# KarelPeeters/kZero

Hardware: AMD Instinct MI355X
Metric: self-play NN evals/sec (node), Chess 20x256 ResNet b=256, 1/2/4/8 GPU (higher is better)
Workload: dtype f16; 1 GPU; chess-20x256 attention head, executor batch 256; engines_per_gpu=1, parallelism=dp1 (no collective)

## Files before the change

### kzero_amd/csrc/kz_decode_dev.hpp

```cpp
#pragma once

struct DecodeDev {
    const int64_t *move_offsets;
    const int32_t *move_indices;
    float *values;
    float *probs;
    int *error_flag;
    int policy_len;
    const uint8_t *sym = nullptr;
    const int32_t *policy_map = nullptr;
    int n_sym = 0;
};

inline DecodeDev decode_dev(const DecodeArgs &a, bool on, int policy_len) {
    return DecodeDev{on ? a.move_offsets : nullptr, a.move_indices, a.values, a.probs, a.error_flag, policy_len, a.sym, a.policy_map, a.n_sym};
}

__device__ __forceinline__ float decode_wave_max_nan(float v) {
#pragma unroll
    for (int off = 32; off > 0; off >>= 1) {
        const float o = __shfl_xor(v, off, 64);
        v = (v != v || o != o) ? NAN : fmaxf(v, o);
    }
    return v;
}

__device__ __forceinline__ void decode_raise(const DecodeDev &d, int board) {
    *reinterpret_cast<volatile int *>(d.error_flag) = 1;
    raise_decode_board(d.error_flag, board);
}

__device__ __forceinline__ float decode_wave_sum(float v) {
#pragma unroll
    for (int off = 32; off > 0; off >>= 1) v += __shfl_xor(v, off, 64);
    return v;
}

template <class LogitAt>
__device__ __forceinline__ void decode_board_wave(const DecodeDev &d, int board, int lane, const float *raw, float *stage,
                                                  int cap, LogitAt logit_at) {
    if (lane == 0) {
        const float s0 = raw[0], s1 = raw[1], s2 = raw[2], s3 = raw[3], s4 = raw[4];
        const float m = fmaxf(s1, fmaxf(s2, s3));
        const float e0 = expf(s1 - m), e1 = expf(s2 - m), e2 = expf(s3 - m), sum = e0 + e1 + e2;
        float *v = d.values + (size_t)board * 5;
        v[0] = tanhf(s0);
        v[1] = e0 / sum;
        v[2] = e1 / sum;
        v[3] = e2 / sum;
        v[4] = s4;
        if (!(sum > 0.0f)) decode_raise(d, board);
    }
    const int64_t lo = d.move_offsets[board];
    const int n = (int)(d.move_offsets[board + 1] - lo);
    const int32_t *pmap = nullptr;
    if (d.sym) {
        const int id = d.sym[board];
        if (id < d.n_sym) pmap = d.policy_map + (size_t)id * d.policy_len;
        else if (lane == 0) decode_raise(d, board);
    }
    if (n <= 0) return;
    auto logit_of = [&](int i) {
        int idx = d.move_indices[lo + i];
        if (d.sym) idx = (pmap && idx >= 0 && idx < d.policy_len) ? pmap[idx] : -1;
        return (idx >= 0 && idx < d.policy_len) ? logit_at(idx) : NAN;
    };
    float mx = -INFINITY;
    for (int i = lane; i < n; i += 64) {
        const float v = logit_of(i);
        if (i < cap) stage[i] = v;
        mx = (mx != mx || v != v) ? NAN : fmaxf(mx, v);
    }
    mx = decode_wave_max_nan(mx);
    float sum = 0.0f;
    for (int i = lane; i < n; i += 64) {
        const float e = expf((i < cap ? stage[i] : logit_of(i)) - mx);
        if (i < cap) stage[i] = e;
        sum += e;
    }
    sum = decode_wave_sum(sum);
    if (lane == 0 && !(sum > 0.0f)) decode_raise(d, board);
    for (int i = lane; i < n; i += 64) d.probs[lo + i] = (i < cap ? stage[i] : expf(logit_of(i) - mx)) / sum;
}
```

### kzero_amd/csrc/kz_encode_dev.hpp

```cpp
#pragma once

__device__ __forceinline__ float encoded_plane(const PackedBoards in, int board, int ch, int square, int hw) {
    float f = 0.0f;
    if (ch < in.n_scalar) {
        f = in.scalars[(size_t)board * in.n_scalar + ch];
    } else if (ch < in.n_scalar + in.n_bool) {
        const uint8_t *bb = in.bits + (size_t)board * in.stride;
        if (in.sym) square = in.square_src[min((int)in.sym[board], in.n_sym - 1) * hw + square];
        const unsigned bit = (unsigned)(ch - in.n_scalar) * hw + square;
        f = (float)((bb[bit >> 3] >> (bit & 7)) & 1);
    }
    return f;
}
```

### kzero_amd/csrc/kz_engine.hip

```cpp
#include <hip/hip_runtime.h>

#include <algorithm>
#include <cmath>
#include <cstdio>
#include <cstdlib>
#include <cstring>
#include <map>
#include <memory>
#include <mutex>
#include <stdexcept>
#include <string>
#include <tuple>
#include <vector>

#include "../../include/kz_hip.h"
#include "kz_kernels.hpp"
#include "kz_model.hpp"

namespace {

#include "kz_engine_util.hpp"
#include "kz_plan.hpp"
#include "kz_device_weights.hpp"

#include "kz_engine_state.hpp"
#include "kz_engine_forward.hpp"

static void experiment_switches(const Model &m, int dtype, int cin_p, PathPlan &p) {
#ifdef KZ_EXPERIMENTS
    const auto env_int = [](const char *name) { return getenv(name) ? atoi(getenv(name)) : 0; };
    if (env_on("KZ_NO_TOWER_F16") && p.tower == Tower::resident_f16) {
        p.tower = kz::tower_split_supported(m.h, m.w, m.channels, m.depth, m.c_in, false) ? Tower::resident_f16g : Tower::conv_igemm;
        p.heads = p.wide = false;
    }
    p.nb4 = p.tower == Tower::resident_f16 && env_int("KZ_TOWER_NB") == 4 && cin_p == 32;
    if (p.nb4) p.heads = false;
    p.tower_prev = p.tower == Tower::resident_f16 && !p.nb4 && env_on("KZ_TOWER_PREV");
    p.t32_dense3 = p.tower == Tower::resident_f32 && env_int("KZ_T32_BOARDS") == 3 &&
                   kz::tower32_dense3_supported((int)m.policy_kind, m.policy_extra_moves, m.policy_conv_channels, m.h, m.w, m.channels,
                                                m.sh_conv.cout, m.sh_fc0.out, p.heads);
    p.att_heads = !p.heads && att_heads_one_launch(m, dtype);
    p.conv2 = env_on("KZ_BOARD_CONV2") && p.tower == Tower::board_conv_f16 &&
              kz::board_conv2_supported(dtype, m.h, m.w, m.channels, m.channels);
    p.graph = env_on("KZ_HIP_GRAPH") && !p.heads;
    p.no_zero_copy = env_on("KZ_NO_ZERO_COPY");
#endif
}

static void launch_geometry_of(const Model &m, const PathPlan &p, int dtype, int batch, int *workgroups, int *boards_per_workgroup) {
    const int cin_p = round_up(m.c_in, 32), cp = round_up(m.channels, 32);
    int per = 0, wgs = 0;
    switch (p.tower) {
// ... 1468 lines not shown
    return guarded("kz_memcpy_d2h", [&]() -> int {
        HIP_TRY(hipSetDevice(device));
        HIP_TRY(hipMemcpy(dst, src, bytes, hipMemcpyDeviceToHost));
        return 0;
    });
}

KZ_API int kz_device_synchronize(int device) {
    return guarded("kz_device_synchronize", [&]() -> int {
        HIP_TRY(hipSetDevice(device));
        HIP_TRY(hipDeviceSynchronize());
        return 0;
    });
}

KZ_API int kz_engine_set_profiling(kz_engine *e, int enable) {
    return guarded("kz_engine_set_profiling", [&]() -> int {
        if (!e) return fail("kz_engine_set_profiling: null engine");
        HIP_TRY(hipSetDevice(e->device));
        if (e->sync_all()) return 1;
        e->prof.clear();
        e->prof.on = enable != 0;
        return 0;
    });
}

KZ_API int kz_engine_kernel_time(kz_engine *e, const char *prefix, double *total_ms, int64_t *launches) {
    return guarded("kz_engine_kernel_time", [&]() -> int {
        if (!e || !prefix || !total_ms || !launches) return fail("kz_engine_kernel_time: null argument");
        HIP_TRY(hipSetDevice(e->device));
// ... 55 lines not shown
```

### kzero_amd/csrc/kz_engine_forward.hpp

```cpp
#pragma once

inline int kz_engine::conv(const Pass &p, const DevConv &w, const void *x, int ldx, void *y, int ldy, int M, int relu, const void *res, bool post,
         int h, int wd, int group, int src_group, int src_off, float *y32, int ldy32) {
    if (w.bws) {
        kz::BoardConvArgs b{};
        b.x = x; b.ldx = 2 * ldx; b.weights = w.bws; b.bias = w.b; b.res = res; b.y = y; b.ldy = 2 * ldy;
        b.y32 = y32; b.ldy32 = ldy32;
        b.post_scale = post ? wts->post_scale : nullptr;
        b.post_shift = post ? wts->post_shift : nullptr;
        b.boards = M / (h * wd); b.h = h; b.w = wd; b.cin = w.cin_p; b.cout = w.cout; b.relu = relu;
        return launch(p, "kz_board_conv_split16", [&] { kz::launch_board_conv_split(b, p.stream); });
    }
    if (w.bw) {
        kz::BoardConvArgs b{};
        b.x = x; b.ldx = ldx; b.weights = w.bw; b.bias = w.b; b.res = res; b.y = y; b.ldy = ldy;
        b.post_scale = post ? wts->post_scale : nullptr;
        b.post_shift = post ? wts->post_shift : nullptr;
        b.boards = M / (h * wd); b.h = h; b.w = wd; b.cin = w.cin_p; b.cout = w.cout; b.relu = relu;
        b.rowmap = wts->bc_rowmap; b.halo = wts->bc_halo; b.n_halo = wts->bc_n_halo;
        return launch(p, "kz_board_conv_f16", [&] {
#ifdef KZ_EXPERIMENTS
            if (w.bw2) kz::launch_board_conv2(b, p.stream);
            else
#endif
// ... 61 lines not shown
        t.x0 = x_in; t.cin_p = cin_p; t.w_stem = wts->res.w_stem; t.w_tower = wts->res.w_tower;
        t.bias = wts->res.bias; t.post_scale = wts->post_scale; t.post_shift = wts->post_shift;
        t.y = act[0]; t.batch = batch; t.h = m.h; t.w = m.w; t.depth = m.depth;
        t.boards_per_wg = plan.tower_nb;
        t.fused_heads = plan.heads;
        t.sh_w0 = wts->sh.w0; t.sh_b0 = wts->sh.b0; t.sh_w1 = wts->sh.w1; t.sh_b1 = wts->sh.b1;
        t.sh_w2 = wts->sh.w2; t.sh_b2 = wts->sh.b2; t.att_idx = wts->res.att_idx;
        t.scalars = d_scalars; t.policy = d_policy;
        t.nonfinite_flag = p.nf_flag; t.epoch = p.nf_epoch;
        if (dec && plan.heads) t.decode = *dec;
        if (tap_out) {
            t.taps = taps();
            range_site = 2 * m.depth + 1;
        }
#ifdef KZ_EXPERIMENTS
        t.prev = plan.tower_prev;
#endif
        if (launch(p, "kz_tower_resident_f16", [&] {
#ifdef KZ_EXPERIMENTS
                if (plan.nb4) kz::launch_tower_resident4(t, xres, p.stream);
                else
#endif
                kz::launch_tower_resident(t, p.stream);
            }))
            return 1;
        tower_out = 0;
        return 0;
    }
    if (!per_layer(plan)) {
        kz::Tower32Args t{};
        t.x0 = (const float *)x_in; t.ldx0 = cin_p; t.c_in = m.c_in; t.weights = wts->res.w32; t.bias = wts->res.bias;
// ... 231 lines not shown
```

### kzero_amd/csrc/kz_kernels.hpp

```cpp
#pragma once
#include <vector>
#include <hip/hip_runtime.h>

#include <cstdint>

namespace kz {

inline int round_up(int v, int m) { return (v + m - 1) / m * m; }

constexpr int ERR_HDR = 4;
inline size_t error_flag_words(int max_batch) { return ERR_HDR + 2 * (size_t)max_batch; }
__device__ __forceinline__ void raise_nonfinite_board(int *nonfinite_flag, int epoch, int board) {
    *reinterpret_cast<volatile int *>(nonfinite_flag - 1 - board) = epoch;
}
__device__ __forceinline__ void raise_decode_board(int *error_flag, int board) {
    *reinterpret_cast<volatile int *>(error_flag + ERR_HDR + 2 * board) = 1;
}

struct PackedBoards {
    const uint8_t *bits = nullptr;
    size_t stride = 0;
    const float *scalars = nullptr;
    int n_scalar = 0, n_bool = 0;
    int n_sym = 0;
// ... 364 lines not shown
    const void *w_stem;
    const void *w_tower;
    const float *bias;
    const float *post_scale, *post_shift;
    void *y;
    int batch, h, w, depth;
    int boards_per_wg;
    bool fused_heads;
    const float *sh_w0, *sh_b0, *sh_w1, *sh_b1, *sh_w2, *sh_b2;
    const int32_t *att_idx;
    float *scalars, *policy;
    int *nonfinite_flag;
    int epoch;
    DecodeArgs decode;
    bool prev;
    TapOut taps;
};
bool tower_resident_supported(int dtype, int h, int w, int channels, int depth, int c_in);
bool tower_heads_supported(int policy_kind, int query_channels, int policy_len, int sh_channels, int sh_size);
size_t tower_packed_weight_elems(int cin_p, int depth);
size_t tower_heads_weight_elems();
size_t tower_weight_pad_elems();
void tower_pack_heads(const float *w_bulk, const float *b_bulk, const float *w_under, const float *b_under,
                      uint16_t *dst, float *bias5);
void tower_pack_weights(const float *oihw, int cout, int cin, int cin_p, uint16_t *dst, bool tap_major = false);
void launch_tower_resident(const TowerArgs &a, hipStream_t stream);
size_t tower4_scratch_bytes(int batch);
void launch_tower_resident4(const TowerArgs &a, void *xres, hipStream_t stream);

}
```

### kzero_amd/csrc/kz_plan.hpp

```cpp
#pragma once


enum class Tower {
    dense_net,
    att_valu,
    att_mfma,
    resident_f16,
    resident_f32,
    resident_split16,
    resident_f16g,
    resident_bf16g,
    resident_i8,
    board_conv_f16,
    board_conv_split16,
    conv_igemm,
};

struct PathPlan {
    Tower tower = Tower::conv_igemm;
    bool heads = false;
    bool wide = false;
    int wide_cap = 0;
    bool att_heads = false;
    bool keep = false;
    int tower_nb = 2;
    int launches = 0;
#ifdef KZ_EXPERIMENTS
    bool nb4 = false, tower_prev = false, t32_dense3 = false, conv2 = false, graph = false, no_zero_copy = false;
#endif
};

bool split_arithmetic(Tower t) { return t == Tower::resident_split16 || t == Tower::board_conv_split16; }
bool split_arithmetic(const PathPlan &p) { return split_arithmetic(p.tower); }

enum class StreamHeads { none, attention, conv };
struct WeightsSpec {
    Tower tower = Tower::conv_igemm;
    StreamHeads heads = StreamHeads::none;
    bool att_heads = false;
    bool conv2 = false, nb4 = false;
    auto fields() const { return std::tie(tower, heads, att_heads, conv2, nb4); }
    bool operator<(const WeightsSpec &o) const { return fields() < o.fields(); }
};
// ... 241 lines not shown
```

### kzero_amd/csrc/kz_tower.hip

```cpp
#include <cstdlib>
#include <type_traits>
#include <vector>

#include "kz_kernels.hpp"
#include "kz_launch.hpp"
#include "kz_tower_boundary.hpp"
namespace kz {

typedef _Float16 h16;
typedef h16 h16x8 __attribute__((ext_vector_type(8)));
typedef h16 h16x4 __attribute__((ext_vector_type(4)));
typedef float f32x4 __attribute__((ext_vector_type(4)));

namespace {

#include "kz_decode_dev.hpp"
#include "kz_encode_dev.hpp"

constexpr int C = 256;
constexpr int RS = C * 2 + 16;
constexpr int URS = 3 * C * 2 + 16;
constexpr int KSTEPS = 72;
constexpr int HEAD_KSTEPS = 5 * 8;
constexpr int POLICY = 1880, LOGIT_LD = 96;
constexpr int TOWER_PF_MAX = 8;

struct TowerDev {
    const h16 *x0;
    const uint4 *w_stem, *w_tower;
    const float *bias, *post_scale, *post_shift;
    h16 *y;
    int cin_p, batch, depth;
    PackedBoards in;
    const float *sh_w0, *sh_b0, *sh_w1, *sh_b1, *sh_w2, *sh_b2;
    const int32_t *att_idx;
    union { float *scalars; unsigned char *tap_base; }; union { float *policy; size_t tap_site_bytes; };
    int *nonfinite_flag;
    int epoch;
    DecodeDev dec;
};

template <int I, int N, class F>
__device__ __forceinline__ void static_for(F &&f) {
    if constexpr (I < N) {
        f(std::integral_constant<int, I>{});
        static_for<I + 1, N>(f);
    }
}

template <int NB>
struct Layout {
    static constexpr int M = NB * 64;
    static constexpr int MT = M / 16;
    static constexpr bool LINE_TILES = NB == 2;
    static constexpr int BPAD = LINE_TILES ? 128 : 0;
    static constexpr int BOARD = 64 * RS + BPAD;
    static constexpr int TS = LINE_TILES ? 8 * RS : 16 * RS;
    static constexpr int IMG = NB * BOARD;
    static constexpr int X_OFF = 0;
    static constexpr int Y_OFF = IMG;
    static constexpr int Z_OFF = 2 * IMG;
    static_assert(Z_OFF % 256 == 0, "zero rows keep the slot pattern of the image rows");
    static constexpr int S_OFF = Z_OFF + 16 * RS;
    static constexpr int TOWER_BYTES = S_OFF + M * 64;
    static constexpr int U_OFF = Z_OFF;
    static constexpr int ACT_OFF = U_OFF + 16 * URS;
    static constexpr int HID_OFF = ACT_OFF + NB * 256 * 4;
    static constexpr int HEADS_BYTES = HID_OFF + NB * 32 * 4;
    static constexpr int LOG_OFF = Y_OFF;
    static constexpr int BYTES = TOWER_BYTES > HEADS_BYTES ? TOWER_BYTES : HEADS_BYTES;
    static_assert(NB * 64 * LOGIT_LD * 4 <= IMG, "logits fit the Y region");
    static constexpr int row_off(int b, int p) { return b * BOARD + p * RS; }
    static_assert(BYTES <= 160 * 1024, "LDS budget");
};

constexpr int SG_VALU = 0x2, SG_SALU = 0x4, SG_MFMA = 0x8, SG_VMEM_READ = 0x20, SG_DS_READ = 0x100;

template <int NB, bool HEADS, int PF, bool WIDE = false, bool PREV = false, bool TAP = false>
__global__ __launch_bounds__(256, 1) void kz_tower_resident(TowerDev a) {
    using L = Layout<NB>;
    constexpr int M = L::M, MT = L::MT;
    static_assert(PF <= TOWER_PF_MAX, "the refills past the end of the stream must land in its padding"); static_assert(!TAP || (!HEADS && !PREV), "the tap instances are the plain tower's");
    extern __shared__ __attribute__((aligned(16))) unsigned char lds[];

    const int tid = threadIdx.x;
    const int wave = __builtin_amdgcn_readfirstlane(tid >> 6);
    const int lane = tid & 63;
    const int fr = lane & 15, kq = lane >> 4;
    const int board0 = blockIdx.x * NB;
    const int layers = 2 * a.depth;
    const int total_ksteps = layers * KSTEPS + (HEADS ? HEAD_KSTEPS : 0);
    const int bias_rows = layers + (HEADS ? 5 : 0);

    const uint4 *wp = a.w_tower + wave * 256 + lane;
    auto wload_prev = [&](int gk, int nt) __attribute__((always_inline)) { return wp[(size_t)gk * 1024 + nt * 64]; };
    typedef const __attribute__((address_space(1))) unsigned char *gptr;
    gptr wk = (gptr)a.w_tower + wave * 4096;
    const unsigned wlane = lane * 16;
    auto wload = [&](gptr k, int nt) __attribute__((always_inline)) {
        typedef unsigned u32x4 __attribute__((ext_vector_type(4)));
        return __builtin_bit_cast(uint4, *reinterpret_cast<const __attribute__((address_space(1))) u32x4 *>(k + wlane + nt * 1024));
    };
    uint4 wreg[PF][4];
#pragma unroll
    for (int s = 0; s < PF; s++) {
        const int g = s < total_ksteps ? s : total_ksteps - 1;
#pragma unroll
        for (int nt = 0; nt < 4; nt++) wreg[s][nt] = PREV ? wload_prev(g, nt) : wload(wk + s * 16384, nt);
    }
    wk += PF * 16384;
    int g = 0;
    auto ring_take = [&](int stage, h16x8 (&af)[4]) __attribute__((always_inline)) {
#pragma unroll
        for (int nt = 0; nt < 4; nt++) af[nt] = *reinterpret_cast<const h16x8 *>(&wreg[stage][nt]);
#ifndef KZ_TW_NO_WLOAD
        if constexpr (PREV) {
            const int gn = g + PF < total_ksteps ? g + PF : total_ksteps - 1;
#pragma unroll
            for (int nt = 0; nt < 4; nt++) wreg[stage][nt] = wload_prev(gn, nt);
        } else {
#pragma unroll
            for (int nt = 0; nt < 4; nt++) wreg[stage][nt] = wload(wk, nt);
        }
#endif
        wk += 16384;
        if constexpr (!PREV) asm("" : "+s"(wk));
    };

    const int sc = WIDE ? a.cin_p >> 5 : 1;
    const int stem_off = WIDE ? L::Y_OFF : L::S_OFF, srow = 64 * sc, spieces = 4 * sc;
    for (int id = tid; id < 16 * RS / 16; id += 256)
        *reinterpret_cast<uint4 *>(lds + L::Z_OFF + id * 16) = make_uint4(0, 0, 0, 0);
    for (int id = tid; id < M * spieces; id += 256) {
        const int row = WIDE ? id / spieces : id >> 2, c = id - row * spieces;
        const int board = board0 + (row >> 6);
        uint4 v = make_uint4(0, 0, 0, 0);
        if (board < a.batch) {
            if (a.in.bits) {
                h16x8 e;
#pragma unroll
                for (int j = 0; j < 8; j++) e[j] = (h16)encoded_plane(a.in, board, c * 8 + j, row & 63, 64);
                v = *reinterpret_cast<const uint4 *>(&e);
            } else {
                v = *reinterpret_cast<const uint4 *>(a.x0 + ((size_t)board0 * 64 + row) * a.cin_p + c * 8);
            }
        }
        *reinterpret_cast<uint4 *>(lds + stem_off + row * srow + c * 16) = v;
    }
    __syncthreads();

    f32x4 acc[4][MT];
    f32x4 bias_next[4];
    auto fetch_bias = [&](int row) __attribute__((always_inline)) {
        const int l = row <= bias_rows ? row : bias_rows;
#pragma unroll
        for (int nt = 0; nt < 4; nt++)
            bias_next[nt] = *reinterpret_cast<const f32x4 *>(a.bias + l * C + wave * 64 + nt * 16 + kq * 4);
    };
    auto init_acc = [&]() __attribute__((always_inline)) {
#pragma unroll
        for (int nt = 0; nt < 4; nt++)
#pragma unroll
            for (int mt = 0; mt < MT; mt++) acc[nt][mt] = bias_next[nt];
    };
    f32x4 post_s[4], post_t[4];
#pragma unroll
    for (int nt = 0; nt < 4; nt++) {
        post_s[nt] = f32x4{1.f, 1.f, 1.f, 1.f};
        post_t[nt] = f32x4{0.f, 0.f, 0.f, 0.f};
    }

    auto relu4 = [](f32x4 v) {
        typedef int i32x4 __attribute__((ext_vector_type(4)));
        i32x4 b = __builtin_bit_cast(i32x4, v);
#pragma unroll
        for (int j = 0; j < 4; j++) b[j] = b[j] > 0 ? b[j] : 0;
        return __builtin_bit_cast(f32x4, b);
    };
    auto to_h4 = [](f32x4 v) { return h16x4{(h16)v[0], (h16)v[1], (h16)v[2], (h16)v[3]}; };
// ... 21 lines not shown
                if constexpr (decltype(post)::value) v = v * post_s[nt] + post_t[nt];
                *reinterpret_cast<h16x4 *>(lds + dst_off + off) = to_h4(v); if constexpr (TAP) tap_put(a, site, tap_chess_live<L::LINE_TILES>(board0, fr, a.batch), tap_chess_row<L::LINE_TILES>(board0, fr, mt) * C + wave * 64 + nt * 16 + kq * 4, to_h4(v));
            }
        }
    };
    constexpr std::true_type YES{};
    constexpr std::false_type NO{};

    const bool x_is0 = (lane & 7) == 0, x_is7 = (lane & 7) == 7, yo_is0 = (lane & 8) == 0, yo_is1 = !yo_is0;
    auto tap_ok = [&](int mt, int dy, int dx) __attribute__((always_inline)) {
        const bool kill_x = (dx < 0 && x_is0) || (dx > 0 && x_is7);
        if constexpr (L::LINE_TILES) return !(kill_x || (dy < 0 && mt == 0) || (dy > 0 && mt == MT - 1));
        else return !(kill_x || ((mt & 3) == 0 && dy < 0 && yo_is0) || ((mt & 3) == 3 && dy > 0 && yo_is1));
    };

    fetch_bias(0);
    init_acc();
    fetch_bias(1);
    for (int ks = 0; ks < 9 * sc; ks++) {
        const int tap = WIDE ? ks / sc : ks, chunk = ks - tap * sc;
        const int dy = tap / 3 - 1, dx = tap % 3 - 1;
        h16x8 af[4];
#pragma unroll
        for (int nt = 0; nt < 4; nt++) {
            const uint4 t = a.w_stem[((ks * 4 + wave) * 4 + nt) * 64 + lane];
            af[nt] = *reinterpret_cast<const h16x8 *>(&t);
        }
#pragma unroll
        for (int mt = 0; mt < MT; mt++) {
            const bool ok = tap_ok(mt, dy, dx);
            const int p = L::LINE_TILES ? (fr >> 3) * 64 + mt * 8 + (fr & 7) : mt * 16 + fr;
            const int off = ok ? stem_off + (p + dy * 8 + dx) * srow + chunk * 64 + kq * 16 : L::Z_OFF + kq * 16;
            const h16x8 bf = *reinterpret_cast<const h16x8 *>(lds + off);
#pragma unroll
            for (int nt = 0; nt < 4; nt++)
                acc[nt][mt] = __builtin_amdgcn_mfma_f32_16x16x32_f16(af[nt], bf, acc[nt][mt], 0, 0, 0);
        }
    }
    epilogue(L::X_OFF, NO, NO, NO);
    __syncthreads();

    const int kq_off = 256 * (kq & 1) + 128 * (kq >> 1);
    const int frag_base = lane_row + kq_off;
    auto tap_rows = [&](int dy, int dx, int src_off, int (&T)[MT]) __attribute__((always_inline)) {
        const int shifted = frag_base + src_off + (dy * 8 + dx) * RS;
        const int zrow = L::Z_OFF + ((fr + dy * 8 + dx) & 15) * RS + kq_off;
        const int zrow_odd = L::LINE_TILES ? L::Z_OFF + ((fr + dy * 8 + dx + 8) & 15) * RS + kq_off : zrow;
        if constexpr (PREV) {
#pragma unroll
            for (int mt = 0; mt < MT; mt++) T[mt] = tap_ok(mt, dy, dx) ? shifted + mt * L::TS : ((mt & 1) ? zrow_odd : zrow);
        } else {
            int z0 = zrow, z1 = zrow_odd;
            asm("" : "+v"(z0), "+v"(z1));
            const bool kill_x = ((dx < 0) & x_is0) | ((dx > 0) & x_is7);
#pragma unroll
// ... 142 lines not shown
        if constexpr (!LEAN) { init_acc(); fetch_bias(layer + 1); }
        if (layer == layers) {
#pragma unroll
            for (int nt = 0; nt < 4; nt++) {
                const int oc = wave * 64 + nt * 16 + kq * 4;
                post_s[nt] = *reinterpret_cast<const f32x4 *>(a.post_scale + oc);
                post_t[nt] = *reinterpret_cast<const f32x4 *>(a.post_shift + oc);
            }
        }
        if constexpr (LEAN) conv_3x3_lean(is_b ? L::Y_OFF : L::X_OFF, is_b ? L::X_OFF : L::Y_OFF, layer + 1); else conv_3x3(is_b ? L::Y_OFF : L::X_OFF);
        if constexpr (LEAN) { if (!is_b) epilogue_lean(L::Y_OFF, NO, NO); else if (layer != layers) epilogue_lean(L::X_OFF, YES, NO); else epilogue_lean(L::X_OFF, YES, YES); }
        else if (!is_b) epilogue(L::Y_OFF, YES, NO, NO, layer);
        else if (layer != layers) epilogue(L::X_OFF, YES, YES, NO, layer); else epilogue(L::X_OFF, YES, YES, YES, layer);
        __syncthreads();
    }

    if constexpr (!HEADS) {
        for (int id = tid; id < M * 32; id += 256) {
            const int p = id >> 5, c16 = id & 31;
            const int board = board0 + (p >> 6);
            if (board < a.batch) {
                const uint4 v = *reinterpret_cast<const uint4 *>(lds + L::X_OFF + L::row_off(p >> 6, p & 63) + c16 * 16);
                *reinterpret_cast<uint4 *>(a.y + ((size_t)board0 * 64 + p) * C + c16 * 8) = v;
            }
        }
    } else {
        {
            float *act = reinterpret_cast<float *>(lds + L::ACT_OFF);
            for (int o = tid; o < NB * 256; o += 256) {
                const int b = o >> 8, c4 = (o >> 6) & 3, p = o & 63;
// ... 2 lines not shown
                float s = a.sh_b0[c4];
#pragma unroll 4
                for (int i = 0; i < C; i += 8) {
                    const h16x8 xv = *reinterpret_cast<const h16x8 *>(row + i * 2);
                    const f32x4 w0 = *reinterpret_cast<const f32x4 *>(w + i), w1 = *reinterpret_cast<const f32x4 *>(w + i + 4);
#pragma unroll
                    for (int j = 0; j < 4; j++) s += (float)xv[j] * w0[j] + (float)xv[4 + j] * w1[j];
                }
                if (!(fabsf(s) <= 3.0e38f) && a.nonfinite_flag && board0 + b < a.batch) {
                    *reinterpret_cast<volatile int *>(a.nonfinite_flag) = a.epoch;
                    raise_nonfinite_board(a.nonfinite_flag, a.epoch, board0 + b);
                }
                act[o] = fmaxf(s, 0.0f);
            }
        }

        {
            const int tb = L::X_OFF + L::row_off(NB == 2 ? fr >> 3 : 0, 56 + (fr & 7)) + kq_off;
            for (int s = 0; s < 3; s++) {
                f32x4 ua[4];
#pragma unroll
                for (int nt = 0; nt < 4; nt++) ua[nt] = bias_next[nt];
                fetch_bias(layers + 2 + s);
#pragma unroll
                for (int ch = 0; ch < 8; ch++) {
                    const h16x8 bf = *reinterpret_cast<const h16x8 *>(lds + tb + ch * 16);
                    h16x8 af[4];
                    ring_take(ch & (PF - 1), af);
#pragma unroll
                    for (int nt = 0; nt < 4; nt++)
                        ua[nt] = __builtin_amdgcn_mfma_f32_16x16x32_f16(af[nt], bf, ua[nt], 0, 0, 0);
                    g++;
                }
                if (NB == 2 || fr < 8) {
#pragma unroll
                    for (int nt = 0; nt < 4; nt++)
                        *reinterpret_cast<h16x4 *>(lds + L::U_OFF + fr * URS + (256 * s + wave * 64 + nt * 16 + kq * 4) * 2) =
                            to_h4(ua[nt]);
                }
            }
        }

        init_acc();
        fetch_bias(layers + 5);
        conv_1x1(L::X_OFF);
        epilogue(L::Y_OFF, NO, NO, NO);

        init_acc();
        conv_1x1(L::X_OFF);
        __syncthreads();
        epilogue(L::X_OFF, NO, NO, NO);
        __syncthreads();

        {
            const float *act = reinterpret_cast<const float *>(lds + L::ACT_OFF);
            float *hid = reinterpret_cast<float *>(lds + L::HID_OFF);
            if (tid < NB * 128) {
                const int pair = tid >> 2, part = tid & 3, b = pair >> 5, j = pair & 31;
                const float *w = a.sh_w1 + j * 256 + part * 64;
                const float *x = act + b * 256 + part * 64;
                float s = 0.0f;
#pragma unroll 4
                for (int i = 0; i < 64; i += 4) {
                    const f32x4 wv = *reinterpret_cast<const f32x4 *>(w + i), xv = *reinterpret_cast<const f32x4 *>(x + i);
                    s += wv[0] * xv[0] + wv[1] * xv[1] + wv[2] * xv[2] + wv[3] * xv[3];
                }
                s += __shfl_xor(s, 1, 64);
                s += __shfl_xor(s, 2, 64);
                if (part == 0) hid[b * 32 + j] = fmaxf(s + a.sh_b1[j], 0.0f);
            }
        }

        constexpr int IT = NB == 2 ? 2 : 1;
        const int hb = NB == 2 ? wave >> 1 : 0;
        const int it0 = NB == 2 ? (wave & 1) * 2 : wave;
        f32x4 la[IT][6];
        {
            int ja[6], ia[IT];
#pragma unroll
            for (int jt = 0; jt < 4; jt++) ja[jt] = L::X_OFF + L::row_off(hb, jt * 16 + fr) + kq_off;
            ja[4] = L::U_OFF + (hb * 8 + (fr & 7)) * URS + (fr >> 3) * 512 + kq_off;
            ja[5] = L::U_OFF + (hb * 8 + (fr & 7)) * URS + 2 * 512 + kq_off;
#pragma unroll
            for (int ii = 0; ii < IT; ii++) ia[ii] = L::Y_OFF + L::row_off(hb, (it0 + ii) * 16 + fr) + kq_off;
#pragma unroll
            for (int ii = 0; ii < IT; ii++)
#pragma unroll
// ... 11 lines not shown
                    for (int jt = 0; jt < 6; jt++)
                        la[ii][jt] = __builtin_amdgcn_mfma_f32_16x16x32_f16(qa[jt], qb[ii], la[ii][jt], 0, 0, 0);
            }
        }
        __syncthreads();
        {
            const float inv = 1.0f / sqrtf((float)C);
#pragma unroll
            for (int ii = 0; ii < IT; ii++)
#pragma unroll
                for (int jt = 0; jt < 6; jt++) {
                    const int i = (it0 + ii) * 16 + fr, j = jt * 16 + kq * 4;
                    *reinterpret_cast<f32x4 *>(lds + L::LOG_OFF + ((hb * 64 + i) * LOGIT_LD + j) * 4) = la[ii][jt] * inv;
                }
        }
        const bool decode = a.dec.move_offsets != nullptr;
        float *raw = reinterpret_cast<float *>(lds + L::ACT_OFF);
        if (tid < NB * 5) {
            const int b = tid / 5, k = tid % 5;
            const float *hid = reinterpret_cast<const float *>(lds + L::HID_OFF) + b * 32;
            float s = a.sh_b2[k];
            for (int i = 0; i < 32; i++) s += a.sh_w2[k * 32 + i] * hid[i];
            if (decode) raw[b * 8 + k] = s;
            else if (board0 + b < a.batch) a.scalars[(size_t)(board0 + b) * 5 + k] = s;
        }
        __syncthreads();
        if (decode) {
            if (wave < NB && board0 + wave < a.batch) {
                const float *lg = reinterpret_cast<const float *>(lds + L::LOG_OFF) + wave * 64 * LOGIT_LD;
                float *stage = reinterpret_cast<float *>(lds + L::X_OFF + L::row_off(wave, 0));
                decode_board_wave(a.dec, board0 + wave, lane, raw + wave * 8, stage, 64 * RS / 4,
                                  [&](int idx) { return lg[a.att_idx[idx]]; });
            }
        } else {
            for (int b = 0; b < NB; b++) {
                if (board0 + b >= a.batch) break;
                const float *lg = reinterpret_cast<const float *>(lds + L::LOG_OFF) + b * 64 * LOGIT_LD;
                float *pol = a.policy + (size_t)(board0 + b) * POLICY;
                for (int k = tid; k < POLICY; k += 256) pol[k] = lg[a.att_idx[k]];
            }
        }
    }
}

#ifndef KZ_PF_NB1
#define KZ_PF_NB1 4
#endif
#ifndef KZ_PF_NB2
#define KZ_PF_NB2 4
#endif
constexpr int PF_NB1 = KZ_PF_NB1, PF_NB2 = KZ_PF_NB2;

void pack_1x1(const float *w, uint16_t *dst) {
    static const int kq_base[4] = {0, 128, 64, 192};
    for (int chunk = 0; chunk < 8; chunk++)
        for (int wave = 0; wave < 4; wave++)
            for (int nt = 0; nt < 4; nt++)
// ... 56 lines not shown
    std::vector<float> tmp((size_t)256 * 256);
    for (int s = 0; s < 3; s++) {
        for (int q = 0; q < 256; q++) {
            for (int c = 0; c < 256; c++) tmp[(size_t)q * 256 + c] = w_under[(size_t)(3 * q + s) * 256 + c];
            bias5[s * 256 + q] = b_under[3 * q + s];
        }
        pack_1x1(tmp.data(), dst + pass * s);
    }
    pack_1x1(w_bulk, dst + pass * 3);
    pack_1x1(w_bulk + (size_t)256 * 256, dst + pass * 4);
    for (int q = 0; q < 256; q++) {
        bias5[3 * 256 + q] = b_bulk[q];
        bias5[4 * 256 + q] = b_bulk[256 + q];
    }
}

namespace {
template <auto Kernel>
void launch_instance(const TowerDev &d, int grid, int bytes, hipStream_t stream) {
    allow_dynamic_lds<Kernel>(bytes);
    Kernel<<<grid, 256, bytes, stream>>>(d);
}

template <bool PREV>
void launch_chess(const TowerDev &d, const TowerArgs &t, hipStream_t stream) {
    const bool heads = t.fused_heads;
    if constexpr (!PREV) {
        if (t.taps.base && !heads) {
            if (t.cin_p > 32) launch_instance<kz_tower_resident<2, false, PF_NB2, true, false, true>>(d, (t.batch + 1) / 2, Layout<2>::BYTES, stream);
            else if (t.boards_per_wg == 1) launch_instance<kz_tower_resident<1, false, PF_NB1, false, false, true>>(d, t.batch, Layout<1>::BYTES, stream);
// ... 29 lines not shown
    d.batch = t.batch;
    d.depth = t.depth;
    d.in = t.in;
    d.sh_w0 = t.sh_w0; d.sh_b0 = t.sh_b0; d.sh_w1 = t.sh_w1; d.sh_b1 = t.sh_b1; d.sh_w2 = t.sh_w2; d.sh_b2 = t.sh_b2;
    d.att_idx = t.att_idx;
    d.scalars = t.scalars;
    d.policy = t.policy;
    d.nonfinite_flag = t.nonfinite_flag;
    d.epoch = t.epoch;
    d.dec = decode_dev(t.decode, t.fused_heads, POLICY);
    if (t.taps.base && !t.fused_heads) {
        d.tap_base = t.taps.base;
        d.tap_site_bytes = t.taps.site_bytes;
    }
#ifdef KZ_EXPERIMENTS
    if (t.prev) return launch_chess<true>(d, t, stream);
#endif
    launch_chess<false>(d, t, stream);
}

}
```

Before: 528,300 evals/s.

## Prefetch stem weights, board inputs and decode offsets early in resident tower kernel

The resident tower kernel now issues the stem weight loads, the packed board bits and scalars, and the decode move offsets and symmetry ids at kernel start, before the LDS zeroing. It stages the board inputs in LDS as 32-bit words so the stem encoding reads LDS instead of scattered global bytes. It also prefetches the first 64 move indices per board before the policy head so their latency hides behind head compute. The cost is extra registers for the 36 stem weight vectors and staged words under launch_bounds(256,1), plus a more complex encode path. Optional timestamp instrumentation behind an experiment flag is also added.

Result: slower. 521,800 evals/s (-1.2%).

```diff
diff --git a/kzero_amd/csrc/kz_decode_dev.hpp b/kzero_amd/csrc/kz_decode_dev.hpp
--- a/kzero_amd/csrc/kz_decode_dev.hpp
+++ b/kzero_amd/csrc/kz_decode_dev.hpp
@@ -36,9 +36,9 @@
     return v;
 }
 
-template <class LogitAt>
-__device__ __forceinline__ void decode_board_wave(const DecodeDev &d, int board, int lane, const float *raw, float *stage,
-                                                  int cap, LogitAt logit_at) {
+template <class LogitAt, class IndexAt>
+__device__ __forceinline__ void decode_board_list(const DecodeDev &d, int board, int lane, const float *raw, float *stage, int cap,
+                                                  LogitAt logit_at, int64_t lo, int n, int id, IndexAt index_at) {
     if (lane == 0) {
         const float s0 = raw[0], s1 = raw[1], s2 = raw[2], s3 = raw[3], s4 = raw[4];
         const float m = fmaxf(s1, fmaxf(s2, s3));
@@ -51,17 +51,14 @@
         v[4] = s4;
         if (!(sum > 0.0f)) decode_raise(d, board);
     }
-    const int64_t lo = d.move_offsets[board];
-    const int n = (int)(d.move_offsets[board + 1] - lo);
     const int32_t *pmap = nullptr;
     if (d.sym) {
-        const int id = d.sym[board];
         if (id < d.n_sym) pmap = d.policy_map + (size_t)id * d.policy_len;
         else if (lane == 0) decode_raise(d, board);
     }
     if (n <= 0) return;
     auto logit_of = [&](int i) {
-        int idx = d.move_indices[lo + i];
+        int idx = index_at(i);
         if (d.sym) idx = (pmap && idx >= 0 && idx < d.policy_len) ? pmap[idx] : -1;
         return (idx >= 0 && idx < d.policy_len) ? logit_at(idx) : NAN;
     };
@@ -82,3 +79,12 @@
     if (lane == 0 && !(sum > 0.0f)) decode_raise(d, board);
     for (int i = lane; i < n; i += 64) d.probs[lo + i] = (i < cap ? stage[i] : expf(logit_of(i) - mx)) / sum;
 }
+
+template <class LogitAt>
+__device__ __forceinline__ void decode_board_wave(const DecodeDev &d, int board, int lane, const float *raw, float *stage,
+                                                  int cap, LogitAt logit_at) {
+    const int64_t lo = d.move_offsets[board];
+    const int n = (int)(d.move_offsets[board + 1] - lo);
+    const int id = d.sym ? d.sym[board] : 0;
+    decode_board_list(d, board, lane, raw, stage, cap, logit_at, lo, n, id, [&](int i) { return d.move_indices[lo + i]; });
+}
diff --git a/kzero_amd/csrc/kz_encode_dev.hpp b/kzero_amd/csrc/kz_encode_dev.hpp
--- a/kzero_amd/csrc/kz_encode_dev.hpp
+++ b/kzero_amd/csrc/kz_encode_dev.hpp
@@ -12,3 +12,15 @@
     }
     return f;
 }
+
+__device__ __forceinline__ int encoded_square(const PackedBoards in, int sym_id , int square, int hw) {
+    return in.sym ? in.square_src[min(sym_id, in.n_sym - 1) * hw + square] : square;
+}
+__device__ __forceinline__ float encoded_plane_staged(const PackedBoards in, const unsigned char *stg, int bits_bytes, int ch,
+                                                      int square, int hw) {
+    const bool is_scalar = ch < in.n_scalar, is_bool = !is_scalar && ch < in.n_scalar + in.n_bool;
+    const float s = reinterpret_cast<const float *>(stg + bits_bytes)[is_scalar ? ch : 0];
+    const unsigned bit = is_bool ? (unsigned)(ch - in.n_scalar) * hw + square : 0u;
+    const float b = (float)((stg[bit >> 3] >> (bit & 7)) & 1);
+    return is_scalar ? s : is_bool ? b : 0.0f;
+}
diff --git a/kzero_amd/csrc/kz_engine.hip b/kzero_amd/csrc/kz_engine.hip
--- a/kzero_amd/csrc/kz_engine.hip
+++ b/kzero_amd/csrc/kz_engine.hip
@@ -36,6 +36,7 @@
     p.nb4 = p.tower == Tower::resident_f16 && env_int("KZ_TOWER_NB") == 4 && cin_p == 32;
     if (p.nb4) p.heads = false;
     p.tower_prev = p.tower == Tower::resident_f16 && !p.nb4 && env_on("KZ_TOWER_PREV");
+    p.tower_stamp = p.tower == Tower::resident_f16 && !p.nb4 && !p.tower_prev && env_on("KZ_TOWER_STAMP");
     p.t32_dense3 = p.tower == Tower::resident_f32 && env_int("KZ_T32_BOARDS") == 3 &&
                    kz::tower32_dense3_supported((int)m.policy_kind, m.policy_extra_moves, m.policy_conv_channels, m.h, m.w, m.channels,
                                                 m.sh_conv.cout, m.sh_fc0.out, p.heads);
@@ -1534,6 +1535,17 @@
     });
 }
 
+#ifdef KZ_EXPERIMENTS
+KZ_API int kz_exp_tower_stamps(int device, unsigned long long *dst, size_t words, size_t *copied, int *kept, int *wgs, int *slots) {
+    return guarded("kz_exp_tower_stamps", [&]() -> int {
+        if (!dst || !copied || !kept || !wgs || !slots) return fail("kz_exp_tower_stamps: null argument");
+        HIP_TRY(hipSetDevice(device));
+        *copied = kz::tower_stamps_read(dst, words, kept, wgs, slots);
+        return 0;
+    });
+}
+#endif
+
 KZ_API int kz_engine_set_profiling(kz_engine *e, int enable) {
     return guarded("kz_engine_set_profiling", [&]() -> int {
         if (!e) return fail("kz_engine_set_profiling: null engine");
diff --git a/kzero_amd/csrc/kz_engine_forward.hpp b/kzero_amd/csrc/kz_engine_forward.hpp
--- a/kzero_amd/csrc/kz_engine_forward.hpp
+++ b/kzero_amd/csrc/kz_engine_forward.hpp
@@ -99,7 +99,7 @@
             range_site = 2 * m.depth + 1;
         }
 #ifdef KZ_EXPERIMENTS
-        t.prev = plan.tower_prev;
+        t.prev = plan.tower_prev; t.stamp = plan.tower_stamp;
 #endif
         if (launch(p, "kz_tower_resident_f16", [&] {
 #ifdef KZ_EXPERIMENTS
diff --git a/kzero_amd/csrc/kz_kernels.hpp b/kzero_amd/csrc/kz_kernels.hpp
--- a/kzero_amd/csrc/kz_kernels.hpp
+++ b/kzero_amd/csrc/kz_kernels.hpp
@@ -402,6 +402,7 @@
     int epoch;
     DecodeArgs decode;
     bool prev;
+    bool stamp;
     TapOut taps;
 };
 bool tower_resident_supported(int dtype, int h, int w, int channels, int depth, int c_in);
@@ -413,6 +414,9 @@
                       uint16_t *dst, float *bias5);
 void tower_pack_weights(const float *oihw, int cout, int cin, int cin_p, uint16_t *dst, bool tap_major = false);
 void launch_tower_resident(const TowerArgs &a, hipStream_t stream);
+#ifdef KZ_EXPERIMENTS
+size_t tower_stamps_read(unsigned long long *dst, size_t words, int *kept, int *wgs, int *slots);
+#endif
 size_t tower4_scratch_bytes(int batch);
 void launch_tower_resident4(const TowerArgs &a, void *xres, hipStream_t stream);
 
diff --git a/kzero_amd/csrc/kz_plan.hpp b/kzero_amd/csrc/kz_plan.hpp
--- a/kzero_amd/csrc/kz_plan.hpp
+++ b/kzero_amd/csrc/kz_plan.hpp
@@ -26,7 +26,7 @@
     int tower_nb = 2;
     int launches = 0;
 #ifdef KZ_EXPERIMENTS
-    bool nb4 = false, tower_prev = false, t32_dense3 = false, conv2 = false, graph = false, no_zero_copy = false;
+    bool nb4 = false, tower_prev = false, tower_stamp = false, t32_dense3 = false, conv2 = false, graph = false, no_zero_copy = false;
 #endif
 };
 
diff --git a/kzero_amd/csrc/kz_tower.hip b/kzero_amd/csrc/kz_tower.hip
--- a/kzero_amd/csrc/kz_tower.hip
+++ b/kzero_amd/csrc/kz_tower.hip
@@ -24,6 +24,7 @@
 constexpr int HEAD_KSTEPS = 5 * 8;
 constexpr int POLICY = 1880, LOGIT_LD = 96;
 constexpr int TOWER_PF_MAX = 8;
+#include "kz_tower_stamps.hpp"
 
 struct TowerDev {
     const h16 *x0;
@@ -38,6 +39,9 @@
     int *nonfinite_flag;
     int epoch;
     DecodeDev dec;
+#ifdef KZ_EXPERIMENTS
+    unsigned long long *stamps;
+#endif
 };
 
 template <int I, int N, class F>
@@ -66,7 +70,9 @@
     static constexpr int U_OFF = Z_OFF;
     static constexpr int ACT_OFF = U_OFF + 16 * URS;
     static constexpr int HID_OFF = ACT_OFF + NB * 256 * 4;
-    static constexpr int HEADS_BYTES = HID_OFF + NB * 32 * 4;
+    static constexpr int DEC_OFF = HID_OFF + NB * 32 * 4;
+    static constexpr int HEADS_BYTES = DEC_OFF + 64;
+    static_assert(DEC_OFF >= TOWER_BYTES && DEC_OFF % 8 == 0 && (NB + 1) * 8 <= 32, "the decode's words are nobody else's");
     static constexpr int LOG_OFF = Y_OFF;
     static constexpr int BYTES = TOWER_BYTES > HEADS_BYTES ? TOWER_BYTES : HEADS_BYTES;
     static_assert(NB * 64 * LOGIT_LD * 4 <= IMG, "logits fit the Y region");
@@ -76,12 +82,13 @@
 
 constexpr int SG_VALU = 0x2, SG_SALU = 0x4, SG_MFMA = 0x8, SG_VMEM_READ = 0x20, SG_DS_READ = 0x100;
 
-template <int NB, bool HEADS, int PF, bool WIDE = false, bool PREV = false, bool TAP = false>
+template <int NB, bool HEADS, int PF, bool WIDE = false, bool PREV = false, bool TAP = false, bool STAMP = false>
 __global__ __launch_bounds__(256, 1) void kz_tower_resident(TowerDev a) {
     using L = Layout<NB>;
     constexpr int M = L::M, MT = L::MT;
     static_assert(PF <= TOWER_PF_MAX, "the refills past the end of the stream must land in its padding"); static_assert(!TAP || (!HEADS && !PREV), "the tap instances are the plain tower's");
     extern __shared__ __attribute__((aligned(16))) unsigned char lds[];
+    KZ_TW_STAMPS_BEGIN();
 
     const int tid = threadIdx.x;
     const int wave = __builtin_amdgcn_readfirstlane(tid >> 6);
@@ -92,6 +99,7 @@
     const int total_ksteps = layers * KSTEPS + (HEADS ? HEAD_KSTEPS : 0);
     const int bias_rows = layers + (HEADS ? 5 : 0);
 
+#include "kz_tower_ends_body.hpp"
     const uint4 *wp = a.w_tower + wave * 256 + lane;
     auto wload_prev = [&](int gk, int nt) __attribute__((always_inline)) { return wp[(size_t)gk * 1024 + nt * 64]; };
     typedef const __attribute__((address_space(1))) unsigned char *gptr;
@@ -109,6 +117,7 @@
         for (int nt = 0; nt < 4; nt++) wreg[s][nt] = PREV ? wload_prev(g, nt) : wload(wk + s * 16384, nt);
     }
     wk += PF * 16384;
+    KZ_TW_STAMP(1);
     int g = 0;
     auto ring_take = [&](int stage, h16x8 (&af)[4]) __attribute__((always_inline)) {
 #pragma unroll
@@ -127,16 +136,36 @@
         if constexpr (!PREV) asm("" : "+s"(wk));
     };
 
+    f32x4 acc[4][MT];
+    f32x4 bias_next[4];
+    auto fetch_bias = [&](int row) __attribute__((always_inline)) {
+        const int l = row <= bias_rows ? row : bias_rows;
+#pragma unroll
+        for (int nt = 0; nt < 4; nt++)
+            bias_next[nt] = *reinterpret_cast<const f32x4 *>(a.bias + l * C + wave * 64 + nt * 16 + kq * 4);
+    };
+    auto init_acc = [&]() __attribute__((always_inline)) {
+#pragma unroll
+        for (int nt = 0; nt < 4; nt++)
+#pragma unroll
+            for (int mt = 0; mt < MT; mt++) acc[nt][mt] = bias_next[nt];
+    };
+    fetch_bias(0);
+    stem_weights_issue();
+    boards_issue();
     const int sc = WIDE ? a.cin_p >> 5 : 1;
     const int stem_off = WIDE ? L::Y_OFF : L::S_OFF, srow = 64 * sc, spieces = 4 * sc;
     for (int id = tid; id < 16 * RS / 16; id += 256)
         *reinterpret_cast<uint4 *>(lds + L::Z_OFF + id * 16) = make_uint4(0, 0, 0, 0);
+    boards_to_lds();
+    __syncthreads();
     for (int id = tid; id < M * spieces; id += 256) {
         const int row = WIDE ? id / spieces : id >> 2, c = id - row * spieces;
         const int board = board0 + (row >> 6);
         uint4 v = make_uint4(0, 0, 0, 0);
         if (board < a.batch) {
-            if (a.in.bits) {
+            if (staged) v = staged_piece(row, c);
+            else if (a.in.bits) {
                 h16x8 e;
 #pragma unroll
                 for (int j = 0; j < 8; j++) e[j] = (h16)encoded_plane(a.in, board, c * 8 + j, row & 63, 64);
@@ -148,21 +177,8 @@
         *reinterpret_cast<uint4 *>(lds + stem_off + row * srow + c * 16) = v;
     }
     __syncthreads();
-
-    f32x4 acc[4][MT];
-    f32x4 bias_next[4];
-    auto fetch_bias = [&](int row) __attribute__((always_inline)) {
-        const int l = row <= bias_rows ? row : bias_rows;
-#pragma unroll
-        for (int nt = 0; nt < 4; nt++)
-            bias_next[nt] = *reinterpret_cast<const f32x4 *>(a.bias + l * C + wave * 64 + nt * 16 + kq * 4);
-    };
-    auto init_acc = [&]() __attribute__((always_inline)) {
-#pragma unroll
-        for (int nt = 0; nt < 4; nt++)
-#pragma unroll
-            for (int mt = 0; mt < MT; mt++) acc[nt][mt] = bias_next[nt];
-    };
+    KZ_TW_STAMP(2);
+
     f32x4 post_s[4], post_t[4];
 #pragma unroll
     for (int nt = 0; nt < 4; nt++) {
@@ -214,31 +230,8 @@
         else return !(kill_x || ((mt & 3) == 0 && dy < 0 && yo_is0) || ((mt & 3) == 3 && dy > 0 && yo_is1));
     };
 
-    fetch_bias(0);
-    init_acc();
-    fetch_bias(1);
-    for (int ks = 0; ks < 9 * sc; ks++) {
-        const int tap = WIDE ? ks / sc : ks, chunk = ks - tap * sc;
-        const int dy = tap / 3 - 1, dx = tap % 3 - 1;
-        h16x8 af[4];
-#pragma unroll
-        for (int nt = 0; nt < 4; nt++) {
-            const uint4 t = a.w_stem[((ks * 4 + wave) * 4 + nt) * 64 + lane];
-            af[nt] = *reinterpret_cast<const h16x8 *>(&t);
-        }
-#pragma unroll
-        for (int mt = 0; mt < MT; mt++) {
-            const bool ok = tap_ok(mt, dy, dx);
-            const int p = L::LINE_TILES ? (fr >> 3) * 64 + mt * 8 + (fr & 7) : mt * 16 + fr;
-            const int off = ok ? stem_off + (p + dy * 8 + dx) * srow + chunk * 64 + kq * 16 : L::Z_OFF + kq * 16;
-            const h16x8 bf = *reinterpret_cast<const h16x8 *>(lds + off);
-#pragma unroll
-            for (int nt = 0; nt < 4; nt++)
-                acc[nt][mt] = __builtin_amdgcn_mfma_f32_16x16x32_f16(af[nt], bf, acc[nt][mt], 0, 0, 0);
-        }
-    }
-    epilogue(L::X_OFF, NO, NO, NO);
-    __syncthreads();
+#include "kz_tower_stem_body.hpp"
+    KZ_TW_STAMP(3);
 
     const int kq_off = 256 * (kq & 1) + 128 * (kq >> 1);
     const int frag_base = lane_row + kq_off;
@@ -411,6 +404,7 @@
         else if (layer != layers) epilogue(L::X_OFF, YES, YES, NO, layer); else epilogue(L::X_OFF, YES, YES, YES, layer);
         __syncthreads();
     }
+    KZ_TW_STAMP(4);
 
     if constexpr (!HEADS) {
         for (int id = tid; id < M * 32; id += 256) {
@@ -443,6 +437,7 @@
                 act[o] = fmaxf(s, 0.0f);
             }
         }
+        KZ_TW_STAMP(5);
 
         {
             const int tb = L::X_OFF + L::row_off(NB == 2 ? fr >> 3 : 0, 56 + (fr & 7)) + kq_off;
@@ -469,6 +464,7 @@
                 }
             }
         }
+        KZ_TW_STAMP(6);
 
         init_acc();
         fetch_bias(layers + 5);
@@ -480,6 +476,7 @@
         __syncthreads();
         epilogue(L::X_OFF, NO, NO, NO);
         __syncthreads();
+        KZ_TW_STAMP(7);
 
         {
             const float *act = reinterpret_cast<const float *>(lds + L::ACT_OFF);
@@ -500,6 +497,8 @@
             }
         }
 
+        decode_prefetch();
+
         constexpr int IT = NB == 2 ? 2 : 1;
         const int hb = NB == 2 ? wave >> 1 : 0;
         const int it0 = NB == 2 ? (wave & 1) * 2 : wave;
@@ -541,7 +540,6 @@
                     *reinterpret_cast<f32x4 *>(lds + L::LOG_OFF + ((hb * 64 + i) * LOGIT_LD + j) * 4) = la[ii][jt] * inv;
                 }
         }
-        const bool decode = a.dec.move_offsets != nullptr;
         float *raw = reinterpret_cast<float *>(lds + L::ACT_OFF);
         if (tid < NB * 5) {
             const int b = tid / 5, k = tid % 5;
@@ -552,12 +550,13 @@
             else if (board0 + b < a.batch) a.scalars[(size_t)(board0 + b) * 5 + k] = s;
         }
         __syncthreads();
+        KZ_TW_STAMP(8);
         if (decode) {
             if (wave < NB && board0 + wave < a.batch) {
                 const float *lg = reinterpret_cast<const float *>(lds + L::LOG_OFF) + wave * 64 * LOGIT_LD;
                 float *stage = reinterpret_cast<float *>(lds + L::X_OFF + L::row_off(wave, 0));
-                decode_board_wave(a.dec, board0 + wave, lane, raw + wave * 8, stage, 64 * RS / 4,
-                                  [&](int idx) { return lg[a.att_idx[idx]]; });
+                decode_staged(raw + wave * 8, stage, 64 * RS / 4,
+                              [&](int idx) { return lg[a.att_idx[idx]]; });
             }
         } else {
             for (int b = 0; b < NB; b++) {
@@ -567,7 +566,18 @@
                 for (int k = tid; k < POLICY; k += 256) pol[k] = lg[a.att_idx[k]];
             }
         }
-    }
+        KZ_TW_STAMP(9);
+    }
+#ifdef KZ_EXPERIMENTS
+    if constexpr (STAMP) {
+        KZ_TW_STAMP(10);
+        KZ_TW_RSTAMP(12);
+        if (lane == 0) {
+#pragma unroll
+            for (int s = 0; s < STAMP_SLOTS; s++) a.stamps[((size_t)blockIdx.x * 4 + wave) * STAMP_SLOTS + s] = st[s];
+        }
+    }
+#endif
 }
 
 #ifndef KZ_PF_NB1
@@ -654,6 +664,24 @@
         bias5[4 * 256 + q] = b_bulk[256 + q];
     }
 }
+
+#ifdef KZ_EXPERIMENTS
+namespace {
+constexpr int STAMP_KEPT = 8, STAMP_WGS = 1024;
+constexpr size_t STAMP_LAUNCH_WORDS = (size_t)STAMP_WGS * 4 * STAMP_SLOTS;
+unsigned long long *g_stamp_buf = nullptr;
+unsigned g_stamp_launches = 0;
+}
+
+size_t tower_stamps_read(unsigned long long *dst, size_t words, int *kept, int *wgs, int *slots) {
+    *kept = STAMP_KEPT; *wgs = STAMP_WGS; *slots = STAMP_SLOTS;
+    if (!g_stamp_buf || !dst) return 0;
+    const size_t n = words < STAMP_KEPT * STAMP_LAUNCH_WORDS ? words : STAMP_KEPT * STAMP_LAUNCH_WORDS;
+    if (hipDeviceSynchronize() != hipSuccess || hipMemcpy(dst, g_stamp_buf, n * 8, hipMemcpyDeviceToHost) != hipSuccess) return 0;
+    (void)hipMemset(g_stamp_buf, 0, STAMP_KEPT * STAMP_LAUNCH_WORDS * 8);
+    return n;
+}
+#endif
 
 namespace {
 template <auto Kernel>
@@ -713,6 +741,14 @@
         d.tap_site_bytes = t.taps.site_bytes;
     }
 #ifdef KZ_EXPERIMENTS
+    if (t.stamp && t.fused_heads && t.cin_p <= 32 && t.boards_per_wg == 2 && !t.prev && (t.batch + 1) / 2 <= STAMP_WGS) {
+        if (!g_stamp_buf && (hipMalloc((void **)&g_stamp_buf, STAMP_KEPT * STAMP_LAUNCH_WORDS * 8) != hipSuccess ||
+                             hipMemset(g_stamp_buf, 0, STAMP_KEPT * STAMP_LAUNCH_WORDS * 8) != hipSuccess)) g_stamp_buf = nullptr;
+        if (g_stamp_buf) {
+            d.stamps = g_stamp_buf + (size_t)(g_stamp_launches++ % STAMP_KEPT) * STAMP_LAUNCH_WORDS;
+            return launch_instance<kz_tower_resident<2, true, PF_NB2, false, false, false, true>>(d, (t.batch + 1) / 2, Layout<2>::BYTES, stream);
+        }
+    }
     if (t.prev) return launch_chess<true>(d, t, stream);
 #endif
     launch_chess<false>(d, t, stream);
diff --git a/kzero_amd/csrc/kz_tower_ends_body.hpp b/kzero_amd/csrc/kz_tower_ends_body.hpp
--- /dev/null
+++ b/kzero_amd/csrc/kz_tower_ends_body.hpp
@@ -0,0 +1,69 @@
+constexpr int STG_TRIPS = WIDE ? 4 : 1;
+const int stg_bits = a.in.n_bool * 8, stg_per = stg_bits + a.in.n_scalar * 4;
+const bool staged = a.in.bits && ((reinterpret_cast<size_t>(a.in.bits) | a.in.stride | reinterpret_cast<size_t>(a.in.scalars)) & 3) == 0 &&
+                    NB * stg_per <= STG_TRIPS * 256 * 4;
+const bool decode = HEADS && a.dec.move_offsets != nullptr;
+uint32_t stg_v[STG_TRIPS];
+int stg_sym = 0, dec_sym = 0, dec_idx0 = 0;
+int64_t dec_off = 0;
+auto boards_issue = [&]() __attribute__((always_inline)) {
+    if (staged) {
+#pragma unroll
+        for (int k = 0; k < STG_TRIPS; k++) {
+            const int t = (tid + k * 256) * 4, b = t >= stg_per ? 1 : 0, w = t - b * stg_per;
+            stg_v[k] = 0;
+            if (t < NB * stg_per && board0 + b < a.batch)
+                stg_v[k] = w < stg_bits ? *reinterpret_cast<const uint32_t *>(a.in.bits + (size_t)(board0 + b) * a.in.stride + w)
+                                        : *reinterpret_cast<const uint32_t *>(reinterpret_cast<const unsigned char *>(a.in.scalars + (size_t)(board0 + b) * a.in.n_scalar) + (w - stg_bits));
+        }
+        if (a.in.sym && tid < NB && board0 + tid < a.batch) stg_sym = a.in.sym[board0 + tid];
+    }
+    if (decode) {
+        if (tid >= 64 && tid <= 64 + NB && board0 + tid - 64 <= a.batch) dec_off = a.dec.move_offsets[board0 + tid - 64];
+        if (a.dec.sym && tid >= 128 && tid < 128 + NB && board0 + tid - 128 < a.batch) dec_sym = a.dec.sym[board0 + tid - 128];
+    }
+};
+auto boards_to_lds = [&]() __attribute__((always_inline)) {
+    if (staged) {
+#pragma unroll
+        for (int k = 0; k < STG_TRIPS; k++)
+            if ((tid + k * 256) * 4 < NB * stg_per) *reinterpret_cast<uint32_t *>(lds + L::X_OFF + (tid + k * 256) * 4) = stg_v[k];
+        if (tid < NB) *reinterpret_cast<int *>(lds + L::X_OFF + NB * stg_per + tid * 4) = stg_sym;
+    }
+    if (decode) {
+        if (tid >= 64 && tid <= 64 + NB) *reinterpret_cast<int64_t *>(lds + L::DEC_OFF + (tid - 64) * 8) = dec_off;
+        if (tid >= 128 && tid < 128 + NB) *reinterpret_cast<int *>(lds + L::DEC_OFF + 32 + (tid - 128) * 4) = dec_sym;
+    }
+};
+auto staged_piece = [&](int row, int c) __attribute__((always_inline)) {
+    const unsigned char *stg = lds + L::X_OFF + (row >> 6) * stg_per;
+    const int id_sym = *reinterpret_cast<const int *>(lds + L::X_OFF + NB * stg_per + (row >> 6) * 4);
+    const int sq = encoded_square(a.in, id_sym, row & 63, 64);
+    h16x8 e;
+#pragma unroll
+    for (int j = 0; j < 8; j++) e[j] = (h16)encoded_plane_staged(a.in, stg, stg_bits, c * 8 + j, sq, 64);
+    return *reinterpret_cast<const uint4 *>(&e);
+};
+uint4 wstem[WIDE ? 1 : 9][4];
+auto stem_weights_issue = [&]() __attribute__((always_inline)) {
+    if constexpr (!WIDE) {
+#pragma unroll
+        for (int ks = 0; ks < 9; ks++)
+#pragma unroll
+            for (int nt = 0; nt < 4; nt++) wstem[ks][nt] = a.w_stem[((ks * 4 + wave) * 4 + nt) * 64 + lane];
+    }
+};
+auto decode_prefetch = [&]() __attribute__((always_inline)) {
+    if (decode && wave < NB && board0 + wave < a.batch) {
+        const int64_t *offs = reinterpret_cast<const int64_t *>(lds + L::DEC_OFF);
+        const int64_t lo = offs[wave];
+        if (lane < offs[wave + 1] - lo) dec_idx0 = a.dec.move_indices[lo + lane];
+    }
+};
+auto decode_staged = [&](const float *raw, float *stage, int cap, auto logit_at) __attribute__((always_inline)) {
+    const int64_t *offs = reinterpret_cast<const int64_t *>(lds + L::DEC_OFF);
+    const int64_t lo = offs[wave];
+    const int *ids = reinterpret_cast<const int *>(lds + L::DEC_OFF + 32);
+    decode_board_list(a.dec, board0 + wave, lane, raw, stage, cap, logit_at, lo, (int)(offs[wave + 1] - lo), ids[wave],
+                      [&](int i) { return i < 64 ? dec_idx0 : a.dec.move_indices[lo + i]; });
+};
diff --git a/kzero_amd/csrc/kz_tower_stamps.hpp b/kzero_amd/csrc/kz_tower_stamps.hpp
--- /dev/null
+++ b/kzero_amd/csrc/kz_tower_stamps.hpp
@@ -0,0 +1,25 @@
+#pragma once
+
+constexpr int STAMP_SLOTS = 16;
+#ifdef KZ_EXPERIMENTS
+#define KZ_TW_STAMP_ASM(slot, ins)                                                             \
+    do {                                                                                       \
+        if constexpr (STAMP) {                                                                 \
+            unsigned long long t_;                                                             \
+            __builtin_amdgcn_sched_barrier(0);                                                 \
+            asm volatile(ins " %0\n\ts_waitcnt lgkmcnt(0)" : "=s"(t_)::"memory");              \
+            __builtin_amdgcn_sched_barrier(0);                                                 \
+            st[slot] = t_;                                                                     \
+        }                                                                                      \
+    } while (0)
+#define KZ_TW_STAMPS_BEGIN()                                              \
+    [[maybe_unused]] unsigned long long st[STAMP ? STAMP_SLOTS : 1] = {}; \
+    KZ_TW_RSTAMP(11);                                                     \
+    KZ_TW_STAMP(0)
+#define KZ_TW_STAMP(slot) KZ_TW_STAMP_ASM(slot, "s_memtime")
+#define KZ_TW_RSTAMP(slot) KZ_TW_STAMP_ASM(slot, "s_memrealtime")
+#else
+#define KZ_TW_STAMPS_BEGIN() do { } while (0)
+#define KZ_TW_STAMP(slot) do { } while (0)
+#define KZ_TW_RSTAMP(slot) do { } while (0)
+#endif
diff --git a/kzero_amd/csrc/kz_tower_stem_body.hpp b/kzero_amd/csrc/kz_tower_stem_body.hpp
--- /dev/null
+++ b/kzero_amd/csrc/kz_tower_stem_body.hpp
@@ -0,0 +1,31 @@
+init_acc();
+fetch_bias(1);
+auto stem_step = [&](int ks, const uint4 (&wv)[4]) __attribute__((always_inline)) {
+    const int tap = WIDE ? ks / sc : ks, chunk = ks - tap * sc;
+    const int dy = tap / 3 - 1, dx = tap % 3 - 1;
+    h16x8 af[4];
+#pragma unroll
+    for (int nt = 0; nt < 4; nt++) af[nt] = *reinterpret_cast<const h16x8 *>(&wv[nt]);
+#pragma unroll
+    for (int mt = 0; mt < MT; mt++) {
+        const bool ok = tap_ok(mt, dy, dx);
+        const int p = L::LINE_TILES ? (fr >> 3) * 64 + mt * 8 + (fr & 7) : mt * 16 + fr;
+        const int off = ok ? stem_off + (p + dy * 8 + dx) * srow + chunk * 64 + kq * 16 : L::Z_OFF + kq * 16;
+        const h16x8 bf = *reinterpret_cast<const h16x8 *>(lds + off);
+#pragma unroll
+        for (int nt = 0; nt < 4; nt++)
+            acc[nt][mt] = __builtin_amdgcn_mfma_f32_16x16x32_f16(af[nt], bf, acc[nt][mt], 0, 0, 0);
+    }
+};
+if constexpr (!WIDE) {
+    static_for<0, 9>([&](auto ks_tag) __attribute__((always_inline)) { stem_step(decltype(ks_tag)::value, wstem[decltype(ks_tag)::value]); });
+} else {
+    for (int ks = 0; ks < 9 * sc; ks++) {
+        uint4 wv[4];
+#pragma unroll
+        for (int nt = 0; nt < 4; nt++) wv[nt] = a.w_stem[((ks * 4 + wave) * 4 + nt) * 64 + lane];
+        stem_step(ks, wv);
+    }
+}
+epilogue(L::X_OFF, NO, NO, NO);
+__syncthreads();
```
